# SHI-Labs/Prompt-Free-Diffusion

Measured on NVIDIA H100. Metric: 512x512 images/sec @ 50 DDIM steps, higher is better.
Workload: dtype fp16

## Files before the change

include/pfd_b200.h:

```cpp
#ifndef PFD_B200_H_
#define PFD_B200_H_

#include <stdint.h>

#ifdef __cplusplus
extern "C" {
#endif

#define PFD_ABI_VERSION 2
#if defined(__GNUC__)
#define PFD_API __attribute__((visibility("default")))
#else
#define PFD_API
#endif
#define PFD_MAX_SEG 3

enum {
  PFD_ACT_NONE = 0,
  PFD_ACT_SILU = 1,
  PFD_ACT_GELU = 2,
  PFD_ACT_RELU = 3,
  PFD_ACT_GEGLU = 4
};

PFD_API int pfd_version(void);
PFD_API const char* pfd_last_error(void);
PFD_API int64_t pfd_launch_count(void);
PFD_API int pfd_set_option(const char* name, int32_t value);

typedef struct pfd_gemm_desc {
  int32_t nseg;
  int32_t taps[PFD_MAX_SEG];
  int32_t a_c[PFD_MAX_SEG];
  const void* a_ptr[PFD_MAX_SEG];
  int64_t a_sx[PFD_MAX_SEG];
  int64_t a_sy[PFD_MAX_SEG];
  int64_t a_sn[PFD_MAX_SEG];
  int32_t in_w, in_h;
  int32_t stride;
  int32_t W, H, NB;

  const void* b_ptr;
  int32_t N;
  int64_t K;
  int64_t b_batch_stride;

  float alpha;
  int32_t act;
  const void* bias;
  const void* rowadd;
  int64_t rowadd_ld;
  const void* residual;

  void* out;
  int64_t so_n1, so_n0, so_y, so_x, so_c1, so_c0;
  int32_t ndiv, cdiv;
  int32_t bn_force;
  int32_t tap_off;
  void* stream;
} pfd_gemm_desc;

PFD_API int pfd_gemm_f16(const pfd_gemm_desc* d);
PFD_API int pfd_groupnorm_f16(const void* x1, int32_t c1, const void* x2, int32_t c2, int32_t NB,
                      int64_t HW, int32_t groups, const void* gamma, const void* beta, float eps,
                      int32_t silu, void* out, float* ws, int32_t zero_ws, void* stream);

// ... 161 lines not shown
```

pfd_b200/autokl.py:

```python
from __future__ import annotations

from typing import Optional

import torch
import torch.nn as nn

from . import native as nv
from .modules import Container, Conv2d, GroupNorm, pk_conv3, pk_conv3_small, pk_lin, pk_mat, pk_norm


def Normalize(c):
    return GroupNorm(32, c, eps=1e-6, affine=True)


class ResnetBlock(nn.Module):

    def __init__(self, in_channels, out_channels=None):
        super().__init__()
        out_channels = out_channels or in_channels
        self.in_channels, self.out_channels = in_channels, out_channels
        self.norm1 = Normalize(in_channels)
        self.conv1 = Conv2d(in_channels, out_channels, 3, padding=1)
        self.norm2 = Normalize(out_channels)
        self.dropout = nn.Dropout(0.0)
        self.conv2 = Conv2d(out_channels, out_channels, 3, padding=1)
        if in_channels != out_channels:
            self.nin_shortcut = Conv2d(in_channels, out_channels, 1)


class AttnBlock(nn.Module):

# ... 148 lines not shown
        if out_posterior:
            return DiagonalGaussianDistribution(mom, zc)
        noise = torch.randn((B, zc, mom.shape[1], mom.shape[2])).to(mom.device)
        return nv.vae_posterior(mom, zc, noise=noise, scale=post_scale, want=("sample",))["sample"]

    @torch.no_grad()
    def decode(self, z: torch.Tensor, pre_scale: float = 1.0) -> torch.Tensor:
        dec = self.decoder
        B, Cz, H, W = z.shape
        nv.gn_reset()
        zc = nv.nchw_to_nhwc(z if z.dtype == torch.float32 else z.to(torch.float16), cpad=8)
        wq, bq = pk_lin(self.post_quant_conv)
        h = nv.linear(zc.reshape(B * H * W, 8), wq, bq, alpha=pre_scale).reshape(B, H, W, 8)
        w, b = cached_conv_in(dec.conv_in, Cz)
        h = nv.conv3x3_im2col(h, w, b)
        h = run_vae_resnet(dec.mid.block_1, h)
        h = run_vae_attn(dec.mid.attn_1, h)
        h = run_vae_resnet(dec.mid.block_2, h)
        for lvl in reversed(range(dec.num_resolutions)):
            up = dec.up[lvl]
            for rb in up.block:
                h = run_vae_resnet(rb, h)
            if lvl != 0:
                w, b = pk_conv3(up.upsample.conv)
                h = nv.conv3x3(nv.upsample2x(h), w, b)
        g, b = pk_norm(dec.norm_out)
        h = nv.groupnorm(h, g, b, dec.norm_out.eps, silu=True)
        w, b = pk_conv3(dec.conv_out)
        h = nv.conv3x3(h, w, b)
        return nv.nhwc_to_nchw(h, dec.out_ch, mul=0.5, add=0.5, lo=0.0, hi=1.0)

    def forward(self, z):
        return self.decode(z)


class DiagonalGaussianDistribution(object):

    def __init__(self, moments: torch.Tensor, zc: int):
        self._mom, self._zc = moments, zc
        o = nv.vae_posterior(moments, zc, want=("mean", "logvar", "std"))
        self.mean, self.logvar, self.std = o["mean"], o["logvar"], o["std"]
        self.deterministic = False

    def sample(self):
        noise = torch.randn(self.mean.shape).to(self.mean.device)
        return nv.vae_posterior(self._mom, self._zc, noise=noise, want=("sample",))["sample"]

    def mode(self):
# ... 13 lines not shown
```

pfd_b200/csrc/gemm_tc.cu:

```cuda
#include <cuda.h>
#include <cuda_fp16.h>
#include <cuda_runtime.h>
#include <math.h>
#include <string.h>

#include "../../include/pfd_b200.h"
#include "common.h"
#include "ptx.cuh"
#include "wgmma.cuh"

namespace pfd {

constexpr int BM = 128;
constexpr int BK = 64;
constexpr int WG_K = 16;
constexpr int GEMM_THREADS = 384;
constexpr int STAGE_A_BYTES = BM * BK * 2;
constexpr int SMEM_BUDGET = 232448;
constexpr int SMEM_FIXED = 1024 + 256;

struct alignas(64) GemmParams {
  CUtensorMap tmA[PFD_MAX_SEG];
  CUtensorMap tmB;
  int nseg;
  int taps[PFD_MAX_SEG];
  int chunks[PFD_MAX_SEG];
  int a_c[PFD_MAX_SEG];
  int stride;
  int tap_off;
  int bw, bh, bn;
  int tiles_w, tiles_h, tiles_nb, n_tiles;
  int W, H, NB, N;
  int b_batched;
  int num_kb;
  int splits;
  int kb_per_split;
  float* ws;
  float alpha;
  int act;
  const __half* bias;
  const __half* rowadd;
  const __half* residual;
  __half* out;
  long long so_n1, so_n0, so_y, so_x, so_c1, so_c0;
  long long rowadd_ld;
  int ndiv, cdiv;
  int vec_ok;
};

constexpr int STORE_THREADS = 96;

template <int BN>
// ... 63 lines not shown

__device__ __forceinline__ __half2 geglu_pair(const float* v, const float* g, float alpha, uint32_t bv, uint32_t bg) {
  const __half2 a = __floats2half2_rn(fmaf(v[0], alpha, h2lo(bv)), fmaf(v[1], alpha, h2hi(bv)));
  const float2 gf = __half22float2(__floats2half2_rn(fmaf(g[0], alpha, h2lo(bg)), fmaf(g[1], alpha, h2hi(bg))));
  return __hmul2(a, __floats2half2_rn(gelu_sig(gf.x), gelu_sig(gf.y)));
}

struct WorkItem {
  int tile, kb0, kb1, slot;
};
__device__ __forceinline__ bool gemm_work(const GemmParams& p, int wi, int total_tiles, WorkItem& w) {
  const int G = gridDim.x, c = blockIdx.x;
  const int work = c + wi * G;
  if (work >= total_tiles * p.splits) return false;
  w.tile = work % total_tiles;
  w.slot = work / total_tiles;
  w.kb0 = w.slot * p.kb_per_split;
  w.kb1 = min(p.num_kb, w.kb0 + p.kb_per_split);
  return true;
}

struct TileOrigin {
  int x0, y0, n0, lbw, lbh;
};
__device__ __forceinline__ TileOrigin tile_origin(const GemmParams& p, int m_tile) {
  TileOrigin o;
  o.x0 = (m_tile % p.tiles_w) * p.bw;
  o.y0 = ((m_tile / p.tiles_w) % p.tiles_h) * p.bh;
  o.n0 = (m_tile / (p.tiles_w * p.tiles_h)) * p.bn;
  o.lbw = __ffs(p.bw) - 1;
  o.lbh = __ffs(p.bh) - 1;
  return o;
}
struct TileRow {
  int x, y, n;
  bool valid;
};
__device__ __forceinline__ TileRow tile_row(const GemmParams& p, const TileOrigin& o, int row) {
  TileRow r;
  r.x = o.x0 + (row & (p.bw - 1));
  r.y = o.y0 + ((row >> o.lbw) & (p.bh - 1));
  r.n = o.n0 + (row >> (o.lbw + o.lbh));
  r.valid = (r.x < p.W) && (r.y < p.H) && (r.n < p.NB);
  return r;
}
__device__ __forceinline__ long long out_row_off(const GemmParams& p, const TileRow& r) {
  return (long long)(r.n / p.ndiv) * p.so_n1 + (long long)(r.n % p.ndiv) * p.so_n0 + (long long)r.y * p.so_y +
         (long long)r.x * p.so_x;
}
__device__ __forceinline__ long long out_col_off(const GemmParams& p, int c) {
  return p.cdiv >= p.N ? (long long)c * p.so_c0 : (long long)(c / p.cdiv) * p.so_c1 + (long long)(c % p.cdiv) * p.so_c0;
}

template <int BN>
__device__ __forceinline__ void gemm_load_bias(const GemmParams& p, int tile, uint32_t (&bias)[BN / 8]) {
  const int col0 = (tile % p.n_tiles) * BN + 2 * (threadIdx.x & 3);
#pragma unroll
  for (int j = 0; j < BN / 8; ++j) bias[j] = (p.bias && col0 + 8 * j < p.N) ? ldg_h2(p.bias + col0 + 8 * j) : 0u;
}

template <int BN, bool GEGLU>
__device__ __forceinline__ void gemm_stage_tile(const GemmParams& p, const float (&acc)[BN / 2],
                                                const uint32_t (&bias)[BN / 8], int cw, int tile, uint8_t* cbuf) {
  constexpr int C_PITCH = GemmCfg<BN>::C_PITCH;
  const int wl = (threadIdx.x >> 5) & 3, lane = threadIdx.x & 31;
  const int n_tile = tile % p.n_tiles;
  const TileOrigin org = tile_origin(p, tile / p.n_tiles);
  const int n_out = GEGLU ? p.N / 2 : p.N;
  const int col_base = n_tile * (GEGLU ? BN / 2 : BN);
  const int cq = 2 * (lane & 3);
  int rows[2];
// ... 92 lines not shown
#pragma unroll 1
    for (int pass0 = 0; pass0 < NPASS; pass0 += STORE_BATCH) {
#pragma unroll
      for (int b = 0; b < STORE_BATCH; ++b) {
        const int row = r0 + (pass0 + b) * RPP;
        const long long off = (col_ok && row < BM) ? row_off(row) : -1;
        if (off < 0) continue;
        uint4 v = *reinterpret_cast<const uint4*>(src + (pass0 + b) * (RPP * C_PITCH));
        if (add_res) {
          __half2* h = reinterpret_cast<__half2*>(&v);
          const __half2* r = reinterpret_cast<const __half2*>(&res[b]);
#pragma unroll
          for (int k = 0; k < 4; ++k) h[k] = __hadd2(h[k], r[k]);
        }
        *reinterpret_cast<uint4*>(p.out + off) = v;
      }
      if (add_res && pass0 + STORE_BATCH < NPASS) load_batch(pass0 + STORE_BATCH);
    }
  };

  if (line_tile) {
    const int rows_in = p.W - org.x0;
    TileRow first;
    first.x = org.x0; first.y = org.y0; first.n = org.n0;
    const long long base = out_row_off(p, first) + col_off;
    const long long so_x = p.so_x;
    store_rows([&](int row) { return row < rows_in ? base + row * so_x : -1ll; });
  } else {
    store_rows([&](int row) {
      const long long ro = rowoff[row];
      return ro >= 0 ? ro + col_off : -1ll;
    });
  }
}

template <int BN>
__device__ __forceinline__ void gemm_epilogue(const GemmParams& p, const float (&acc)[BN / 2], int cw, int tile,
                                              int split, int m_tiles) {
  const int wl = (threadIdx.x >> 5) & 3, lane = threadIdx.x & 31;
  const int n_tile = tile % p.n_tiles;
  const int m_tile = tile / p.n_tiles;
  const TileOrigin org = tile_origin(p, m_tile);
  const bool geglu = (p.act == PFD_ACT_GEGLU);
  const int n_out = geglu ? p.N / 2 : p.N;
  const int col_base = n_tile * (geglu ? BN / 2 : BN);
  const int cq = 2 * (lane & 3);
  int rows[2];
// ... 89 lines not shown
  const uint32_t bars = base + STAGES * Cfg::STAGE_BYTES + Cfg::C_BYTES;
  auto full_bar = [&](int s) { return bars + 8u * s; };
  auto empty_bar = [&](int s) { return bars + 8u * (STAGES + s); };
  const uint32_t c_full = bars + 16u * STAGES, c_empty = c_full + 8u;

  const int wg = threadIdx.x >> 7;
  const bool staged = p.vec_ok && p.splits == 1;

  if (threadIdx.x == 0) {
    for (int s = 0; s < p.nseg; ++s) tma_prefetch_desc(&p.tmA[s]);
    tma_prefetch_desc(&p.tmB);
    for (int s = 0; s < STAGES; ++s) {
      mbar_init(full_bar(s), 1);
      mbar_init(empty_bar(s), 8);
    }
    mbar_init(c_full, 8);
    mbar_init(c_empty, STORE_THREADS / 32);
    mbar_fence_init();
  }
  __syncthreads();
  pdl_wait();
  pdl_launch_dependents();

  const int m_tiles = p.tiles_w * p.tiles_h * p.tiles_nb;
  const int total_tiles = m_tiles * p.n_tiles;

  if (wg == 0) {
    setmaxnreg_dec<Cfg::PRODUCER_REGS>();
    if (threadIdx.x >= 32 && staged) {
      uint32_t c_phase = 0;
      WorkItem w;
      for (int wi = 0; gemm_work(p, wi, total_tiles, w); ++wi) {
        if (p.act == PFD_ACT_GEGLU) gemm_store_tile<BN, true>(p, w.tile, cbuf, rowoff + (c_phase ? BM : 0), c_full, c_phase);
        else gemm_store_tile<BN, false>(p, w.tile, cbuf, rowoff + (c_phase ? BM : 0), c_full, c_phase);
        __syncwarp();
        if ((threadIdx.x & 31) == 0) mbar_arrive(c_empty);
        c_phase ^= 1u;
      }
    } else if (threadIdx.x == 0) {
      int stage = 0;
      uint32_t phase = 0;
      WorkItem w;
      for (int wi = 0; gemm_work(p, wi, total_tiles, w); ++wi) {
        const int tile = w.tile, kb_begin = w.kb0, kb_end = w.kb1;
        const int n_tile = tile % p.n_tiles;
        const int m_tile = tile / p.n_tiles;
        const int tx = m_tile % p.tiles_w;
        const int ty = (m_tile / p.tiles_w) % p.tiles_h;
        const int tn = m_tile / (p.tiles_w * p.tiles_h);
        const int x0 = tx * p.bw * p.stride;
        const int y0 = ty * p.bh * p.stride;
        const int n0 = tn * p.bn;
        const int bcoord = p.b_batched ? n0 : 0;
        int kofs = 0;
        int kbi = 0;
        for (int s = 0; s < p.nseg; ++s) {
          const int ntap = p.taps[s];
          for (int t = 0; t < ntap; ++t) {
            const int dy = (ntap == 9) ? (t / 3 - 1 + p.tap_off) : 0;
            const int dx = (ntap == 9) ? (t % 3 - 1 + p.tap_off) : 0;
            for (int j = 0; j < p.chunks[s]; ++j, ++kbi) {
              if (kbi < kb_begin || kbi >= kb_end) continue;
              mbar_wait(empty_bar(stage), phase ^ 1u);
              mbar_expect_tx(full_bar(stage), Cfg::STAGE_BYTES);
              tma_load_4d(smemA + stage * STAGE_A_BYTES, &p.tmA[s], full_bar(stage), j * BK, x0 + dx, y0 + dy, n0);
              tma_load_3d(smemB + stage * Cfg::STAGE_B_BYTES, &p.tmB, full_bar(stage), kofs + j * BK, n_tile * BN,
                          bcoord);
              if (++stage == STAGES) {
                stage = 0;
                phase ^= 1u;
              }
            }
            kofs += p.a_c[s];
          }
        }
      }
    }
  } else {
    setmaxnreg_inc<Cfg::CONSUMER_REGS>();
    const int cw = wg - 1;
    const bool arrive_lane = (threadIdx.x & 31) == 0;
    int stage = 0;
    uint32_t phase = 0, c_phase = 0;
// ... 22 lines not shown
        }
      }
      wgmma_wait<0>();
      if (prev >= 0 && arrive_lane) mbar_arrive(empty_bar(prev));
      if (staged) {
        if (!Cfg::BIAS_EARLY) gemm_load_bias<BN>(p, w.tile, bias);
        mbar_wait(c_empty, c_phase ^ 1u);
        if (p.act == PFD_ACT_GEGLU) gemm_stage_tile<BN, true>(p, acc, bias, cw, w.tile, cbuf);
        else gemm_stage_tile<BN, false>(p, acc, bias, cw, w.tile, cbuf);
        __syncwarp();
        if (arrive_lane) mbar_arrive(c_full);
        c_phase ^= 1u;
      } else {
        gemm_epilogue<BN>(p, acc, cw, w.tile, w.slot, m_tiles);
      }
    }
  }
}

__global__ void __launch_bounds__(256)
splitk_finish_kernel(const __grid_constant__ GemmParams p) {
  pdl_wait();
  pdl_launch_dependents();
  const int m_tiles = p.tiles_w * p.tiles_h * p.tiles_nb;
  const long long rows_pad = (long long)m_tiles * BM;
  const int vecs = p.N / 8;
  const long long total = rows_pad * vecs;
  for (long long i = (long long)blockIdx.x * blockDim.x + threadIdx.x; i < total; i += (long long)gridDim.x * blockDim.x) {
    const int v = (int)(i % vecs);
    const long long prow = i / vecs;
    const TileRow r = tile_row(p, tile_origin(p, (int)(prow / BM)), (int)(prow % BM));
    if (!r.valid) continue;
    const int col = v * 8;
    float acc[8];
#pragma unroll
    for (int k = 0; k < 8; ++k) acc[k] = 0.f;
    for (int s = 0; s < p.splits; ++s) {
      const float4* src = reinterpret_cast<const float4*>(p.ws + ((long long)s * rows_pad + prow) * p.N + col);
      const float4 a = __ldg(src), b = __ldg(src + 1);
      acc[0] += a.x; acc[1] += a.y; acc[2] += a.z; acc[3] += a.w;
      acc[4] += b.x; acc[5] += b.y; acc[6] += b.z; acc[7] += b.w;
    }
    uint4 bv = make_uint4(0, 0, 0, 0), rv = bv;
    if (p.bias) bv = __ldg(reinterpret_cast<const uint4*>(p.bias + col));
    if (p.rowadd) rv = __ldg(reinterpret_cast<const uint4*>(p.rowadd + (long long)r.n * p.rowadd_ld + col));
    const uint32_t* b2 = &bv.x;
    const uint32_t* r2 = &rv.x;
// ... 20 lines not shown
        const long long off = row_off + out_col_off(p, col + k);
        __half h = __float2half_rn(acc[k]);
        if (p.residual) h = __hadd(h, p.residual[off]);
        p.out[off] = h;
      }
    }
  }
}

constexpr size_t SPLITK_WS_BYTES = (64ull << 20) - 4096;

static inline long long cdivll(long long a, long long b) { return (a + b - 1) / b; }

template <int BN>
static int launch_gemm(const GemmParams& p, int grid, cudaStream_t stream) {
  using Cfg = GemmCfg<BN>;
  static int trace = -1;
  if (trace < 0) {
    const char* e = getenv("PFD_GEMM_TRACE");
    trace = (e && e[0] == '1') ? 1 : 0;
  }
  if (trace)
    fprintf(stderr, "GEMMTRACE M=%lld N=%d K=%d nseg=%d taps=%d stride=%d act=%d bias=%d res=%d rowadd=%d BN=%d "
            "splits=%d grid=%d batched=%d vec=%d plain=%d\n", (long long)p.W * p.H * p.NB, p.N, p.num_kb * BK,
            p.nseg, p.taps[0], p.stride, p.act, p.bias != nullptr, p.residual != nullptr, p.rowadd != nullptr, BN,
            p.splits, grid, p.b_batched, p.vec_ok, (int)(p.cdiv >= p.N));
  if (int rc = smem_opt_in<gemm_wgmma_kernel<BN>>(Cfg::SMEM_BYTES, "gemm_wgmma_kernel")) return rc;
  launch_k(gemm_wgmma_kernel<BN>, dim3(grid), dim3(GEMM_THREADS), Cfg::SMEM_BYTES, stream, p);
  return check_launch("pfd_gemm_f16");
}

}

using namespace pfd;

extern "C" PFD_API int pfd_gemm_f16(const pfd_gemm_desc* d) {
  if (!d) return set_error("pfd_gemm_f16: null descriptor");
  if (d->nseg < 1 || d->nseg > PFD_MAX_SEG) return set_error("pfd_gemm_f16: nseg %d out of range", d->nseg);
  if (d->N <= 0 || d->N % 8) return set_error("pfd_gemm_f16: N=%d must be a positive multiple of 8", d->N);
  if (d->K % 8) return set_error("pfd_gemm_f16: K pitch %lld must be a multiple of 8", (long long)d->K);
  if (d->W <= 0 || d->H <= 0 || d->NB <= 0) return set_error("pfd_gemm_f16: empty output raster");
  if (d->stride != 1 && d->stride != 2) return set_error("pfd_gemm_f16: stride %d unsupported", d->stride);
  if (d->tap_off != 0 && d->tap_off != 1) return set_error("pfd_gemm_f16: tap_off %d unsupported", d->tap_off);
  if (!d->out || !d->b_ptr) return set_error("pfd_gemm_f16: null out/b pointer");
  long long ktot = 0;
  for (int s = 0; s < d->nseg; ++s) {
    if (d->taps[s] != 1 && d->taps[s] != 9) return set_error("pfd_gemm_f16: taps[%d]=%d", s, d->taps[s]);
    if (d->a_c[s] <= 0 || d->a_c[s] % 8) return set_error("pfd_gemm_f16: a_c[%d]=%d must be a multiple of 8", s, d->a_c[s]);
    if (!d->a_ptr[s]) return set_error("pfd_gemm_f16: a_ptr[%d] is null", s);
    if ((reinterpret_cast<uintptr_t>(d->a_ptr[s]) & 15) || (d->a_sx[s] % 8) || (d->a_sy[s] % 8) || (d->a_sn[s] % 8))
      return set_error("pfd_gemm_f16: A segment %d not 16-byte aligned/strided", s);
    ktot += (long long)d->taps[s] * d->a_c[s];
  }
  if (ktot > d->K) return set_error("pfd_gemm_f16: segments cover K=%lld > pitch %lld", ktot, (long long)d->K);
  if (reinterpret_cast<uintptr_t>(d->b_ptr) & 15) return set_error("pfd_gemm_f16: B not 16-byte aligned");
  const bool geglu = d->act == PFD_ACT_GEGLU;

  GemmParams p;
  memset(&p, 0, sizeof(p));
  p.nseg = d->nseg;
  p.stride = d->stride;
  p.tap_off = d->tap_off;
  p.W = d->W; p.H = d->H; p.NB = d->NB; p.N = d->N;
  p.b_batched = d->b_batch_stride != 0;
  p.alpha = d->alpha;
  p.act = d->act;
  p.bias = static_cast<const __half*>(d->bias);
  p.rowadd = static_cast<const __half*>(d->rowadd);
  p.residual = static_cast<const __half*>(d->residual);
  p.rowadd_ld = d->rowadd_ld > 0 ? d->rowadd_ld : d->N;
  p.out = static_cast<__half*>(d->out);
  p.so_n1 = d->so_n1; p.so_n0 = d->so_n0; p.so_y = d->so_y; p.so_x = d->so_x;
  p.so_c1 = d->so_c1; p.so_c0 = d->so_c0;
  p.ndiv = d->ndiv > 0 ? d->ndiv : 1;
  p.cdiv = d->cdiv > 0 ? d->cdiv : (1 << 30);
  p.vec_ok = (d->so_c0 == 1) && (p.cdiv % 8 == 0) && (d->so_n1 % 8 == 0) && (d->so_n0 % 8 == 0) &&
             (d->so_y % 8 == 0) && (d->so_x % 8 == 0) && (d->so_c1 % 8 == 0) &&
             ((reinterpret_cast<uintptr_t>(d->out) & 15) == 0) &&
             ((reinterpret_cast<uintptr_t>(d->residual) & 15) == 0);
  if ((reinterpret_cast<uintptr_t>(d->bias) & 15) || (reinterpret_cast<uintptr_t>(d->rowadd) & 15) || (d->rowadd_ld % 8))
    return set_error("pfd_gemm_f16: bias/rowadd must be 16-byte aligned");

  int bw = 128, bh = 1, bn = 1;
  if (!p.b_batched) {
    long long best = -1;
    for (int cw = 128; cw >= 1; cw >>= 1) {
      if (cw * d->stride > 256) continue;
      for (int ch = 128 / cw; ch >= 1; ch >>= 1) {
        if (ch * d->stride > 256) continue;
        int cn = 128 / (cw * ch);
        long long cost = cdivll(d->W, cw) * cdivll(d->H, ch) * cdivll(d->NB, cn);
        if (best < 0 || cost < best) {
          best = cost; bw = cw; bh = ch; bn = cn;
        }
      }
    }
  }
  p.bw = bw; p.bh = bh; p.bn = bn;
  p.tiles_w = (int)cdivll(d->W, bw);
  p.tiles_h = (int)cdivll(d->H, bh);
  p.tiles_nb = (int)cdivll(d->NB, bn);
  const long long m_tiles = (long long)p.tiles_w * p.tiles_h * p.tiles_nb;

  bool short_k_plain = !p.b_batched && !geglu;
  int kb_count = 0;
  for (int s = 0; s < d->nseg; ++s) {
    if (d->taps[s] != 1) short_k_plain = false;
    kb_count += d->taps[s] * ((d->a_c[s] + BK - 1) / BK);
  }
  short_k_plain = short_k_plain && kb_count <= 40;
  const int cands[5] = {256, 192, 160, 128, 64};
  int BNsel = 128;
  double best_cost = -1;
  const int sms = plan_sms();
  for (int i = 0; i < 5; ++i) {
    const int bn_c = cands[i];
    if (geglu && (d->N % bn_c)) continue;
    if (d->bn_force && d->bn_force != bn_c) continue;
    if (short_k_plain && !d->bn_force && bn_c != 64) continue;
    const long long nt = cdivll(d->N, bn_c);
    const long long tiles = m_tiles * nt;
    const double waves = (double)cdivll(tiles, sms);
    const double cost = waves * (bn_c + 24);
    if (best_cost < 0 || cost < best_cost - 1e-9) {
      best_cost = cost; BNsel = bn_c;
    }
  }
  if (best_cost < 0) return set_error("pfd_gemm_f16: no valid N tile (bn_force=%d, N=%d, geglu=%d)", d->bn_force, d->N, (int)geglu);
  p.n_tiles = (int)cdivll(d->N, BNsel);
  p.splits = 1;

  int num_kb = 0;
  for (int s = 0; s < d->nseg; ++s) {
    p.taps[s] = d->taps[s];
    p.a_c[s] = d->a_c[s];
    p.chunks[s] = (d->a_c[s] + BK - 1) / BK;
    num_kb += p.taps[s] * p.chunks[s];
    cuuint64_t dims[4] = {(cuuint64_t)d->a_c[s], (cuuint64_t)d->in_w, (cuuint64_t)d->in_h, (cuuint64_t)d->NB};
    cuuint64_t strides[3] = {(cuuint64_t)d->a_sx[s] * 2, (cuuint64_t)d->a_sy[s] * 2, (cuuint64_t)d->a_sn[s] * 2};
    cuuint32_t box[4] = {(cuuint32_t)BK, (cuuint32_t)(bw * d->stride), (cuuint32_t)(bh * d->stride), (cuuint32_t)bn};
    cuuint32_t estr[4] = {1, (cuuint32_t)d->stride, (cuuint32_t)d->stride, 1};
    if (int rc = encode_tensor_map_f16(&p.tmA[s], d->a_ptr[s], 4, dims, strides, box, estr, "A")) return rc;
// ... 11 lines not shown
        break;
      }
    const long long nt_sk = cdivll(d->N, bn_sk);
    const long long tiles_sk = m_tiles * nt_sk;
    if (tiles_sk * 2 <= sms) {
      int splits = (int)(sms / tiles_sk);
      if (splits > 8) splits = 8;
      if (splits > num_kb / 8) splits = num_kb / 8;
      const size_t need = (size_t)splits * (size_t)m_tiles * BM * (size_t)d->N * sizeof(float);
      if (splits >= 2 && need <= SPLITK_WS_BYTES) {
        float* ws = skws;
        if (ws) {
          BNsel = bn_sk;
          p.n_tiles = (int)nt_sk;
          p.splits = splits;
          p.kb_per_split = (num_kb + splits - 1) / splits;
          p.splits = (num_kb + p.kb_per_split - 1) / p.kb_per_split;
          p.ws = ws;
        }
      }
    }
  }
  {
    const long long nbatch = p.b_batched ? d->NB : 1;
    cuuint64_t dims[3] = {(cuuint64_t)d->K, (cuuint64_t)d->N, (cuuint64_t)nbatch};
    const long long bs = p.b_batched ? d->b_batch_stride : (long long)d->K * d->N;
    cuuint64_t strides[2] = {(cuuint64_t)d->K * 2, (cuuint64_t)bs * 2};
    cuuint32_t box[3] = {(cuuint32_t)BK, (cuuint32_t)BNsel, 1};
    cuuint32_t estr[3] = {1, 1, 1};
    if (int rc = encode_tensor_map_f16(&p.tmB, d->b_ptr, 3, dims, strides, box, estr, "B")) return rc;
  }
  const long long total = m_tiles * p.n_tiles * p.splits;
  int grid = (int)(total < sms ? total : sms);
  int rc;
  switch (BNsel) {
    case 64: rc = launch_gemm<64>(p, grid, st); break;
    case 128: rc = launch_gemm<128>(p, grid, st); break;
    case 160: rc = launch_gemm<160>(p, grid, st); break;
    case 192: rc = launch_gemm<192>(p, grid, st); break;
    default: rc = launch_gemm<256>(p, grid, st); break;
  }
  if (rc || p.splits == 1) return rc;
  const long long vec_items = m_tiles * BM * (long long)(d->N / 8);
  long long fgrid = (vec_items + 255) / 256;
  if (fgrid > 8LL * sms) fgrid = 8LL * sms;
  launch_k(splitk_finish_kernel, dim3((unsigned)fgrid), dim3(256), 0, st, p);
  return check_launch("pfd_gemm_f16(split-K finish)");
// ... 2 lines not shown
```

pfd_b200/modules.py:

```python
from __future__ import annotations

from typing import Callable, Optional, Sequence, Tuple

import torch
import torch.nn as nn

from .graphs import generation, watch


class _Holder:
    def forward(self, *a, **k):
        raise RuntimeError(f"{type(self).__name__} is a parameter holder: pfd_b200 computes through "
                           "the CUDA C-ABI kernels only (no torch fallback)")


class Conv2d(_Holder, nn.Conv2d):
    pass


class Linear(_Holder, nn.Linear):
    pass


class GroupNorm(_Holder, nn.GroupNorm):
# ... 68 lines not shown
    o, i, kh, kw = w.shape
    if cin is not None and cin > i:
        w = torch.cat([w, w.new_zeros((o, cin - i, kh, kw))], 1)
    return w.permute(0, 2, 3, 1).reshape(o, -1).contiguous()


def pk_conv3(conv: nn.Conv2d, skip: Optional[nn.Conv2d] = None) -> Tuple[torch.Tensor, Optional[torch.Tensor]]:
    def build():
        w = pack_conv(conv.weight)
        b = fp16(conv.bias)
        if skip is not None:
            ws = fp16(skip.weight).reshape(skip.weight.shape[0], -1)
            w = torch.cat([w, ws], 1).contiguous()
            if skip.bias is not None:
                b = (conv.bias.detach().float() + skip.bias.detach().float()).to(torch.float16).contiguous()
        if w.shape[0] % 8:
            w = pad_rows(w)
            b = pad_rows(b) if b is not None else None
        return w, b
    params = [conv.weight, conv.bias] + ([skip.weight, skip.bias] if skip is not None else [])
    return cached(conv, "conv3" + ("+skip" if skip is not None else ""), params, build)


def pk_conv3_small(conv: nn.Conv2d) -> Tuple[torch.Tensor, Optional[torch.Tensor]]:
    def build():
        w = pad_cols(pack_conv(conv.weight))
        b = fp16(conv.bias)
        if w.shape[0] % 8:
            w, b = pad_rows(w), (pad_rows(b) if b is not None else None)
        return w, b
    return cached(conv, "conv3s", [conv.weight, conv.bias], build)


def pk_mat(mod: nn.Module, weight: torch.Tensor, bias: Optional[torch.Tensor], key: str = "mat",
           rows: Optional[slice] = None) -> Tuple[torch.Tensor, Optional[torch.Tensor]]:
    def build():
        w = fp16(weight).reshape(weight.shape[0], -1)
        b = fp16(bias)
        if rows is not None:
            w = w[rows].contiguous()
            b = b[rows].contiguous() if b is not None else None
        if w.shape[1] % 8:
            w = pad_cols(w)
        if w.shape[0] % 8:
            w, b = pad_rows(w), (pad_rows(b) if b is not None else None)
        return w, b
# ... 14 lines not shown
```

pfd_b200/native.py:

```python
from __future__ import annotations

import ctypes
import os
import re
from ctypes import POINTER, c_char_p, c_float, c_int32, c_int64, c_uint32, c_void_p
from typing import Dict, List, Optional, Sequence, Tuple

import torch

_HERE = os.path.dirname(os.path.abspath(__file__))
LIB_PATH = os.environ.get("PFD_B200_LIB") or os.path.join(_HERE, "libpfd_b200.so")
HEADER = os.path.join(_HERE, os.pardir, "include", "pfd_b200.h")

PFD_MAX_SEG = 3
ACT_NONE, ACT_SILU, ACT_GELU, ACT_RELU, ACT_GEGLU = 0, 1, 2, 3, 4
PFD_KSAMPLER_NCOEF = 6
PFD_HED_MAX_SIDES = 5
PFD_PIDINET_SIDE_PARAMS = 161
PFD_MLSD_TOPK = 200
PFD_OPENPOSE_MAX_PEAKS = 128
PFD_OPENPOSE_MAX_PERSONS = 17 * PFD_OPENPOSE_MAX_PEAKS


class GemmDesc(ctypes.Structure):
    _fields_ = [
        ("nseg", c_int32),
        ("taps", c_int32 * PFD_MAX_SEG),
        ("a_c", c_int32 * PFD_MAX_SEG),
        ("a_ptr", c_void_p * PFD_MAX_SEG),
        ("a_sx", c_int64 * PFD_MAX_SEG),
        ("a_sy", c_int64 * PFD_MAX_SEG),
        ("a_sn", c_int64 * PFD_MAX_SEG),
        ("in_w", c_int32), ("in_h", c_int32),
        ("stride", c_int32),
        ("W", c_int32), ("H", c_int32), ("NB", c_int32),
        ("b_ptr", c_void_p),
        ("N", c_int32),
        ("K", c_int64),
        ("b_batch_stride", c_int64),
        ("alpha", c_float),
        ("act", c_int32),
        ("bias", c_void_p),
        ("rowadd", c_void_p),
        ("rowadd_ld", c_int64),
        ("residual", c_void_p),
        ("out", c_void_p),
        ("so_n1", c_int64), ("so_n0", c_int64), ("so_y", c_int64), ("so_x", c_int64),
        ("so_c1", c_int64), ("so_c0", c_int64),
        ("ndiv", c_int32), ("cdiv", c_int32),
        ("bn_force", c_int32),
        ("tap_off", c_int32),
        ("stream", c_void_p),
    ]


class DevicePtr(c_void_p):

    @classmethod
    def from_param(cls, obj):
        if isinstance(obj, torch.Tensor):
# ... 110 lines not shown
def _chk16(t: torch.Tensor, name: str) -> None:
    if t.dtype != torch.float16 or not t.is_cuda:
        raise RuntimeError(f"{name}: expected a CUDA fp16 tensor, got {t.dtype} on {t.device}")


def _chk32(t: torch.Tensor, name: str) -> None:
    if t.dtype != torch.float32 or not t.is_cuda or not t.is_contiguous():
        raise RuntimeError(f"{name}: expected a contiguous CUDA fp32 tensor, got {t.dtype} on {t.device}")


def _chk_image(x: torch.Tensor, what: str) -> Tuple[torch.Tensor, int]:
    if x.dim() != 4 or x.shape[1] != 3 or not x.is_cuda or x.dtype not in (torch.float16, torch.float32):
        raise RuntimeError(f"{what}: expected a CUDA fp16/fp32 [B,3,H,W] image, got {tuple(x.shape)} {x.dtype} "
                           f"{x.device}")
    return x.contiguous(), int(x.dtype == torch.float32)


def gemm_raw(segs: Sequence[Tuple[torch.Tensor, int, int, Tuple[int, int, int]]], *, in_w: int,
             in_h: int, stride: int, W: int, H: int, NB: int, w: torch.Tensor, N: int, K: int,
             b_batch_stride: int = 0, alpha: float = 1.0, act: int = ACT_NONE,
             bias: Optional[torch.Tensor] = None, rowadd: Optional[torch.Tensor] = None,
             residual: Optional[torch.Tensor] = None, out: torch.Tensor,
             so: Tuple[int, int, int, int, int, int], ndiv: int = 1, cdiv: int = 0,
             bn_force: int = 0, tap_off: int = 0) -> None:
    d = GemmDesc()
    d.nseg = len(segs)
    for i, (t, taps, c, (sx, sy, sn)) in enumerate(segs):
        _chk16(t, f"A[{i}]")
        d.taps[i] = taps
        d.a_c[i] = c
        d.a_ptr[i] = t.data_ptr()
        d.a_sx[i], d.a_sy[i], d.a_sn[i] = sx, sy, sn
    d.in_w, d.in_h, d.stride = in_w, in_h, stride
    d.W, d.H, d.NB = W, H, NB
    _chk16(w, "B")
    d.b_ptr = w.data_ptr()
    d.N, d.K, d.b_batch_stride = N, K, b_batch_stride
    d.alpha, d.act = alpha, act
    d.bias = _p(bias)
    d.rowadd = _p(rowadd)
    d.rowadd_ld = rowadd.stride(0) if rowadd is not None else 0
    d.residual = _p(residual)
    d.out = out.data_ptr()
    d.so_n1, d.so_n0, d.so_y, d.so_x, d.so_c1, d.so_c0 = so
    d.ndiv, d.cdiv = ndiv, cdiv
    d.bn_force = bn_force
    d.tap_off = tap_off
    d.stream = stream_ptr()
    _check(load().pfd_gemm_f16(ctypes.byref(d)), "pfd_gemm_f16")


def linear(x: torch.Tensor, w: torch.Tensor, bias: Optional[torch.Tensor] = None, *, act: int = ACT_NONE,
           residual: Optional[torch.Tensor] = None, out: Optional[torch.Tensor] = None,
           alpha: float = 1.0, x2: Optional[torch.Tensor] = None, bn_force: int = 0) -> torch.Tensor:
    M, K1 = x.shape
    N = w.shape[0]
    n_out = N // 2 if act == ACT_GEGLU else N
    if out is None:
        out = torch.empty((M, n_out), device=x.device, dtype=torch.float16)
    segs = [(x, 1, K1, (x.stride(0), x.stride(0) * M, x.stride(0) * M))]
# ... 21 lines not shown
    tile = torch.arange(n2 // bn, device=w.device).reshape(-1, 1)
    j = torch.arange(h, device=w.device).reshape(1, -1)
    src = torch.stack([tile * h + j, inner + tile * h + j], dim=1).reshape(-1)
    wp = w.index_select(0, src).contiguous()
    bp = b.index_select(0, src).contiguous() if b is not None else None
    return wp, bp, bn


def conv3x3(x: torch.Tensor, w: torch.Tensor, bias: Optional[torch.Tensor] = None, *, stride: int = 1,
            rowadd: Optional[torch.Tensor] = None, act: int = ACT_NONE,
            residual: Optional[torch.Tensor] = None, out: Optional[torch.Tensor] = None,
            skip: Sequence[torch.Tensor] = (), tap_off: int = 0) -> torch.Tensor:
    NB, H, W, C = x.shape
    Ho, Wo = (H - 1 - tap_off) // stride + 1, (W - 1 - tap_off) // stride + 1
    N = w.shape[0]
    if out is None:
        out = torch.empty((NB, Ho, Wo, N), device=x.device, dtype=torch.float16)
    segs = [(x, 9, C, (x.stride(2), x.stride(1), x.stride(0)))]
    for s in skip:
        segs.append((s, 1, s.shape[3], (s.stride(2), s.stride(1), s.stride(0))))
    gemm_raw(segs, in_w=W, in_h=H, stride=stride, W=Wo, H=Ho, NB=NB, w=w, N=N, K=w.stride(0), act=act,
             bias=bias, rowadd=rowadd, residual=residual, out=out,
             so=(out.stride(0), 0, out.stride(1), out.stride(2), 0, 1), tap_off=tap_off)
    return out


def conv1x1(x: torch.Tensor, w: torch.Tensor, bias: Optional[torch.Tensor] = None, *, act: int = ACT_NONE,
            residual: Optional[torch.Tensor] = None, out: Optional[torch.Tensor] = None,
            x2: Optional[torch.Tensor] = None) -> torch.Tensor:
    NB, H, W, C = x.shape
    N = w.shape[0]
    if out is None:
        out = torch.empty((NB, H, W, N), device=x.device, dtype=torch.float16)
    r = residual.reshape(NB * H * W, -1) if residual is not None else None
    linear(x.reshape(NB * H * W, C), w, bias, act=act, residual=r, out=out.reshape(NB * H * W, N),
           x2=None if x2 is None else x2.reshape(NB * H * W, -1))
    return out


def conv1x1_into(x: torch.Tensor, w: torch.Tensor, bias: Optional[torch.Tensor], out: torch.Tensor, *,
                 act: int = ACT_NONE) -> torch.Tensor:
    NB, H, W, C = x.shape
    gemm_raw([(x, 1, C, (x.stride(2), x.stride(1), x.stride(0)))], in_w=W, in_h=H, stride=1, W=W, H=H, NB=NB, w=w,
             N=w.shape[0], K=w.stride(0), act=act, bias=bias, out=out,
             so=(out.stride(0), 0, out.stride(1), out.stride(2), 0, 1))
    return out
# ... 677 lines not shown
```

pfd_b200/unet.py:

```python
from __future__ import annotations

from typing import Dict, List, Optional, Sequence, Tuple

import torch
import torch.nn as nn

from . import native as nv
from . import attention as att
from .attention import attend, ceil8, project_heads, project_heads_fused, project_vt_swapped
from .modules import (Conv2d, GroupNorm, IndexedSequential, LayerNorm, Linear, cached, pk_conv3,
                      pk_conv3_small, pk_lin, pk_mat, pk_norm)


class ResBlock(nn.Module):

    def __init__(self, channels, emb_channels, dropout=0.0, out_channels=None, **_):
        super().__init__()
        self.channels = channels
        self.out_channels = out_channels or channels
        self.in_layers = IndexedSequential(GroupNorm(32, channels), nn.SiLU(),
                                           Conv2d(channels, self.out_channels, 3, padding=1))
        self.emb_layers = IndexedSequential(nn.SiLU(), Linear(emb_channels, self.out_channels))
        self.out_layers = IndexedSequential(GroupNorm(32, self.out_channels), nn.SiLU(), nn.Dropout(p=dropout),
                                            Conv2d(self.out_channels, self.out_channels, 3, padding=1))
        if self.out_channels == channels:
            self.skip_connection = nn.Identity()
        else:
            self.skip_connection = Conv2d(channels, self.out_channels, 1)


class Downsample(nn.Module):

    def __init__(self, channels, out_channels=None):
        super().__init__()
# ... 249 lines not shown
        self.parameter_group = {'global': self.time_embed, 'data': self.data_blocks,
                                'context': self.context_blocks}

    def get_d_head_n_heads(self, ch):
        if self.num_head_channels is None:
            return ch // self.num_heads, self.num_heads
        return self.num_head_channels, ch // self.num_head_channels

    def resblocks(self) -> List[ResBlock]:
        return [blk[0] for blk in self.data_blocks if isinstance(blk[0], ResBlock)]

    def prepare_context(self, context: torch.Tensor) -> List[Tuple[torch.Tensor, torch.Tensor]]:
        return [context_kv(cb[0], context) for cb in self.context_blocks]

    def run_data_block(self, idx: int, h, h2, embs: Dict[int, torch.Tensor]):
        layer = self.data_blocks[idx][0]
        if isinstance(layer, ResBlock):
            return run_resblock(layer, h, h2, embs[idx])
        assert h2 is None
        if isinstance(layer, Downsample):
            w, b = pk_conv3(layer.op)
            return nv.conv3x3(h, w, b, stride=2)
        if isinstance(layer, Upsample):
            w, b = pk_conv3(layer.conv)
            return nv.conv3x3(nv.upsample2x(h), w, b)
        if isinstance(layer, IndexedSequential):
            g, b = pk_norm(layer[0])
            hn = nv.groupnorm(h, g, b, layer[0].eps, silu=True)
            w, bb = pk_conv3(layer[2])
            return nv.conv3x3(hn, w, bb)
        if isinstance(layer, Conv2d):
            w, b = pk_conv3_small(layer)
            return nv.conv3x3_im2col(h, w, b)
        raise RuntimeError(f"unknown data block {type(layer)}")

    def apply(self, x: torch.Tensor, timesteps: torch.Tensor, context: torch.Tensor,
              control: Optional[List[torch.Tensor]] = None,
              kv: Optional[List[Tuple[torch.Tensor, torch.Tensor]]] = None,
              mixed_contexts: Optional[List[Tuple[torch.Tensor, float]]] = None) -> torch.Tensor:
        x = x.to(torch.float16)
        context = context.to(torch.float16).contiguous()
        B = x.shape[0]
        nv.gn_reset()
        silu_emb = time_embed_silu(self.time_embed, timesteps, self.model_channels)
        rbs = [i for i, blk in enumerate(self.data_blocks) if isinstance(blk[0], ResBlock)]
        emb_list = batched_emb_layers(self, [self.data_blocks[i][0] for i in rbs], silu_emb)
        embs = dict(zip(rbs, emb_list))
        if kv is None and mixed_contexts is None:
# ... 36 lines not shown
```

Before: 3.772.

## Fuse nearest upsample into 3x3 conv via four-phase 2x2 folded weights

Replaces the nearest-neighbour upsample followed by a 3x3 conv with a single implicit GEMM. For each of the four output phases, the 3x3 kernel is folded into a 2x2 kernel applied to the low-resolution input, and the phase selects both the weight batch and the output offset. This avoids materialising the 4x-larger upsampled tensor and cuts the conv K dimension from 9 to 4 taps per channel. It also changes the BN heuristic for short-K plain GEMMs (128 when N>=640 with enough tiles) and excludes BN=256 for up2x, and it adds phase indexing overhead to the tile scheduling.

Result: faster. 3.843, median of 6 (+1.9%).

```diff
diff --git a/include/pfd_b200.h b/include/pfd_b200.h
--- a/include/pfd_b200.h
+++ b/include/pfd_b200.h
@@ -42,6 +42,7 @@
 
   const void* b_ptr;
   int32_t N;
+  int32_t up2x;
   int64_t K;
   int64_t b_batch_stride;
 
diff --git a/pfd_b200/autokl.py b/pfd_b200/autokl.py
--- a/pfd_b200/autokl.py
+++ b/pfd_b200/autokl.py
@@ -6,7 +6,7 @@
 import torch.nn as nn
 
 from . import native as nv
-from .modules import Container, Conv2d, GroupNorm, pk_conv3, pk_conv3_small, pk_lin, pk_mat, pk_norm
+from .modules import Container, Conv2d, GroupNorm, pk_conv3, pk_conv3_small, pk_conv3_up2x, pk_lin, pk_mat, pk_norm
 
 
 def Normalize(c):
@@ -201,8 +201,8 @@
             for rb in up.block:
                 h = run_vae_resnet(rb, h)
             if lvl != 0:
-                w, b = pk_conv3(up.upsample.conv)
-                h = nv.conv3x3(nv.upsample2x(h), w, b)
+                w, b = pk_conv3_up2x(up.upsample.conv)
+                h = nv.conv3x3_up2x(h, w, b)
         g, b = pk_norm(dec.norm_out)
         h = nv.groupnorm(h, g, b, dec.norm_out.eps, silu=True)
         w, b = pk_conv3(dec.conv_out)
diff --git a/pfd_b200/csrc/gemm_tc.cu b/pfd_b200/csrc/gemm_tc.cu
--- a/pfd_b200/csrc/gemm_tc.cu
+++ b/pfd_b200/csrc/gemm_tc.cu
@@ -28,6 +28,8 @@
   int a_c[PFD_MAX_SEG];
   int stride;
   int tap_off;
+  int phases;
+  long long ph_sy, ph_sx;
   int bw, bh, bn;
   int tiles_w, tiles_h, tiles_nb, n_tiles;
   int W, H, NB, N;
@@ -137,9 +139,17 @@
 
 struct TileOrigin {
   int x0, y0, n0, lbw, lbh;
+  long long obase;
 };
 __device__ __forceinline__ TileOrigin tile_origin(const GemmParams& p, int m_tile) {
   TileOrigin o;
+  o.obase = 0;
+  if (p.phases > 1) {
+    const int per_phase = p.tiles_w * p.tiles_h * p.tiles_nb;
+    const int ph = m_tile / per_phase;
+    m_tile -= ph * per_phase;
+    o.obase = ((ph & 2) ? p.ph_sy : 0ll) + ((ph & 1) ? p.ph_sx : 0ll);
+  }
   o.x0 = (m_tile % p.tiles_w) * p.bw;
   o.y0 = ((m_tile / p.tiles_w) % p.tiles_h) * p.bh;
   o.n0 = (m_tile / (p.tiles_w * p.tiles_h)) * p.bn;
@@ -150,6 +160,7 @@
 struct TileRow {
   int x, y, n;
   bool valid;
+  long long obase;
 };
 __device__ __forceinline__ TileRow tile_row(const GemmParams& p, const TileOrigin& o, int row) {
   TileRow r;
@@ -157,11 +168,12 @@
   r.y = o.y0 + ((row >> o.lbw) & (p.bh - 1));
   r.n = o.n0 + (row >> (o.lbw + o.lbh));
   r.valid = (r.x < p.W) && (r.y < p.H) && (r.n < p.NB);
+  r.obase = o.obase;
   return r;
 }
 __device__ __forceinline__ long long out_row_off(const GemmParams& p, const TileRow& r) {
-  return (long long)(r.n / p.ndiv) * p.so_n1 + (long long)(r.n % p.ndiv) * p.so_n0 + (long long)r.y * p.so_y +
-         (long long)r.x * p.so_x;
+  return r.obase + (long long)(r.n / p.ndiv) * p.so_n1 + (long long)(r.n % p.ndiv) * p.so_n0 +
+         (long long)r.y * p.so_y + (long long)r.x * p.so_x;
 }
 __device__ __forceinline__ long long out_col_off(const GemmParams& p, int c) {
   return p.cdiv >= p.N ? (long long)c * p.so_c0 : (long long)(c / p.cdiv) * p.so_c1 + (long long)(c % p.cdiv) * p.so_c0;
@@ -300,7 +312,7 @@
   if (line_tile) {
     const int rows_in = p.W - org.x0;
     TileRow first;
-    first.x = org.x0; first.y = org.y0; first.n = org.n0;
+    first.x = org.x0; first.y = org.y0; first.n = org.n0; first.obase = org.obase;
     const long long base = out_row_off(p, first) + col_off;
     const long long so_x = p.so_x;
     store_rows([&](int row) { return row < rows_in ? base + row * so_x : -1ll; });
@@ -436,7 +448,7 @@
   pdl_wait();
   pdl_launch_dependents();
 
-  const int m_tiles = p.tiles_w * p.tiles_h * p.tiles_nb;
+  const int m_tiles = p.tiles_w * p.tiles_h * p.tiles_nb * p.phases;
   const int total_tiles = m_tiles * p.n_tiles;
 
   if (wg == 0) {
@@ -458,21 +470,23 @@
       for (int wi = 0; gemm_work(p, wi, total_tiles, w); ++wi) {
         const int tile = w.tile, kb_begin = w.kb0, kb_end = w.kb1;
         const int n_tile = tile % p.n_tiles;
-        const int m_tile = tile / p.n_tiles;
+        const int per_phase = p.tiles_w * p.tiles_h * p.tiles_nb;
+        const int ph = (tile / p.n_tiles) / per_phase;
+        const int m_tile = (tile / p.n_tiles) % per_phase;
         const int tx = m_tile % p.tiles_w;
         const int ty = (m_tile / p.tiles_w) % p.tiles_h;
         const int tn = m_tile / (p.tiles_w * p.tiles_h);
         const int x0 = tx * p.bw * p.stride;
         const int y0 = ty * p.bh * p.stride;
         const int n0 = tn * p.bn;
-        const int bcoord = p.b_batched ? n0 : 0;
+        const int bcoord = p.b_batched ? n0 : ph;
         int kofs = 0;
         int kbi = 0;
         for (int s = 0; s < p.nseg; ++s) {
           const int ntap = p.taps[s];
           for (int t = 0; t < ntap; ++t) {
-            const int dy = (ntap == 9) ? (t / 3 - 1 + p.tap_off) : 0;
-            const int dx = (ntap == 9) ? (t % 3 - 1 + p.tap_off) : 0;
+            const int dy = (ntap == 9) ? (t / 3 - 1 + p.tap_off) : (ntap == 4) ? (t / 2 - 1 + (ph >> 1)) : 0;
+            const int dx = (ntap == 9) ? (t % 3 - 1 + p.tap_off) : (ntap == 4) ? (t % 2 - 1 + (ph & 1)) : 0;
             for (int j = 0; j < p.chunks[s]; ++j, ++kbi) {
               if (kbi < kb_begin || kbi >= kb_end) continue;
               mbar_wait(empty_bar(stage), phase ^ 1u);
@@ -541,7 +555,7 @@
 splitk_finish_kernel(const __grid_constant__ GemmParams p) {
   pdl_wait();
   pdl_launch_dependents();
-  const int m_tiles = p.tiles_w * p.tiles_h * p.tiles_nb;
+  const int m_tiles = p.tiles_w * p.tiles_h * p.tiles_nb * p.phases;
   const long long rows_pad = (long long)m_tiles * BM;
   const int vecs = p.N / 8;
   const long long total = rows_pad * vecs;
@@ -608,9 +622,9 @@
   }
   if (trace)
     fprintf(stderr, "GEMMTRACE M=%lld N=%d K=%d nseg=%d taps=%d stride=%d act=%d bias=%d res=%d rowadd=%d BN=%d "
-            "splits=%d grid=%d batched=%d vec=%d plain=%d\n", (long long)p.W * p.H * p.NB, p.N, p.num_kb * BK,
-            p.nseg, p.taps[0], p.stride, p.act, p.bias != nullptr, p.residual != nullptr, p.rowadd != nullptr, BN,
-            p.splits, grid, p.b_batched, p.vec_ok, (int)(p.cdiv >= p.N));
+            "splits=%d grid=%d batched=%d vec=%d plain=%d phases=%d\n", (long long)p.W * p.H * p.NB * p.phases, p.N,
+            p.num_kb * BK, p.nseg, p.taps[0], p.stride, p.act, p.bias != nullptr, p.residual != nullptr, p.rowadd != nullptr, BN,
+            p.splits, grid, p.b_batched, p.vec_ok, (int)(p.cdiv >= p.N), p.phases);
   if (int rc = smem_opt_in<gemm_wgmma_kernel<BN>>(Cfg::SMEM_BYTES, "gemm_wgmma_kernel")) return rc;
   launch_k(gemm_wgmma_kernel<BN>, dim3(grid), dim3(GEMM_THREADS), Cfg::SMEM_BYTES, stream, p);
   return check_launch("pfd_gemm_f16");
@@ -628,10 +642,17 @@
   if (d->W <= 0 || d->H <= 0 || d->NB <= 0) return set_error("pfd_gemm_f16: empty output raster");
   if (d->stride != 1 && d->stride != 2) return set_error("pfd_gemm_f16: stride %d unsupported", d->stride);
   if (d->tap_off != 0 && d->tap_off != 1) return set_error("pfd_gemm_f16: tap_off %d unsupported", d->tap_off);
+  if (d->up2x != 0 && d->up2x != 1) return set_error("pfd_gemm_f16: up2x %d unsupported", d->up2x);
+  if (d->up2x && (d->stride != 1 || d->tap_off != 0 || d->b_batch_stride != 0 || d->W != 2 * d->in_w ||
+                  d->H != 2 * d->in_h))
+    return set_error("pfd_gemm_f16: up2x needs stride 1, tap_off 0, shared weights and W, H = 2 in_w, 2 in_h "
+                     "(got stride %d, tap_off %d, W %d, H %d, in_w %d, in_h %d)", d->stride, d->tap_off, d->W, d->H,
+                     d->in_w, d->in_h);
   if (!d->out || !d->b_ptr) return set_error("pfd_gemm_f16: null out/b pointer");
   long long ktot = 0;
   for (int s = 0; s < d->nseg; ++s) {
-    if (d->taps[s] != 1 && d->taps[s] != 9) return set_error("pfd_gemm_f16: taps[%d]=%d", s, d->taps[s]);
+    if (d->up2x ? d->taps[s] != 4 : (d->taps[s] != 1 && d->taps[s] != 9))
+      return set_error("pfd_gemm_f16: taps[%d]=%d (up2x %d)", s, d->taps[s], d->up2x);
     if (d->a_c[s] <= 0 || d->a_c[s] % 8) return set_error("pfd_gemm_f16: a_c[%d]=%d must be a multiple of 8", s, d->a_c[s]);
     if (!d->a_ptr[s]) return set_error("pfd_gemm_f16: a_ptr[%d] is null", s);
     if ((reinterpret_cast<uintptr_t>(d->a_ptr[s]) & 15) || (d->a_sx[s] % 8) || (d->a_sy[s] % 8) || (d->a_sn[s] % 8))
@@ -647,7 +668,9 @@
   p.nseg = d->nseg;
   p.stride = d->stride;
   p.tap_off = d->tap_off;
-  p.W = d->W; p.H = d->H; p.NB = d->NB; p.N = d->N;
+  p.phases = d->up2x ? 4 : 1;
+  const int sc = d->up2x ? 2 : 1;
+  p.W = d->W / sc; p.H = d->H / sc; p.NB = d->NB; p.N = d->N;
   p.b_batched = d->b_batch_stride != 0;
   p.alpha = d->alpha;
   p.act = d->act;
@@ -656,7 +679,9 @@
   p.residual = static_cast<const __half*>(d->residual);
   p.rowadd_ld = d->rowadd_ld > 0 ? d->rowadd_ld : d->N;
   p.out = static_cast<__half*>(d->out);
-  p.so_n1 = d->so_n1; p.so_n0 = d->so_n0; p.so_y = d->so_y; p.so_x = d->so_x;
+  p.so_n1 = d->so_n1; p.so_n0 = d->so_n0; p.so_y = d->so_y * sc; p.so_x = d->so_x * sc;
+  p.ph_sy = d->up2x ? d->so_y : 0;
+  p.ph_sx = d->up2x ? d->so_x : 0;
   p.so_c1 = d->so_c1; p.so_c0 = d->so_c0;
   p.ndiv = d->ndiv > 0 ? d->ndiv : 1;
   p.cdiv = d->cdiv > 0 ? d->cdiv : (1 << 30);
@@ -675,7 +700,7 @@
       for (int ch = 128 / cw; ch >= 1; ch >>= 1) {
         if (ch * d->stride > 256) continue;
         int cn = 128 / (cw * ch);
-        long long cost = cdivll(d->W, cw) * cdivll(d->H, ch) * cdivll(d->NB, cn);
+        long long cost = cdivll(p.W, cw) * cdivll(p.H, ch) * cdivll(d->NB, cn);
         if (best < 0 || cost < best) {
           best = cost; bw = cw; bh = ch; bn = cn;
         }
@@ -683,10 +708,10 @@
     }
   }
   p.bw = bw; p.bh = bh; p.bn = bn;
-  p.tiles_w = (int)cdivll(d->W, bw);
-  p.tiles_h = (int)cdivll(d->H, bh);
+  p.tiles_w = (int)cdivll(p.W, bw);
+  p.tiles_h = (int)cdivll(p.H, bh);
   p.tiles_nb = (int)cdivll(d->NB, bn);
-  const long long m_tiles = (long long)p.tiles_w * p.tiles_h * p.tiles_nb;
+  const long long m_tiles = (long long)p.tiles_w * p.tiles_h * p.tiles_nb * p.phases;
 
   bool short_k_plain = !p.b_batched && !geglu;
   int kb_count = 0;
@@ -695,6 +720,7 @@
     kb_count += d->taps[s] * ((d->a_c[s] + BK - 1) / BK);
   }
   short_k_plain = short_k_plain && kb_count <= 40;
+  const int short_k_bn = (!d->residual && d->N >= 640 && m_tiles >= 64) ? 128 : 64;
   const int cands[5] = {256, 192, 160, 128, 64};
   int BNsel = 128;
   double best_cost = -1;
@@ -703,7 +729,8 @@
     const int bn_c = cands[i];
     if (geglu && (d->N % bn_c)) continue;
     if (d->bn_force && d->bn_force != bn_c) continue;
-    if (short_k_plain && !d->bn_force && bn_c != 64) continue;
+    if (short_k_plain && !d->bn_force && bn_c != short_k_bn) continue;
+    if (d->up2x && !d->bn_force && bn_c == 256) continue;
     const long long nt = cdivll(d->N, bn_c);
     const long long tiles = m_tiles * nt;
     const double waves = (double)cdivll(tiles, sms);
@@ -761,7 +788,7 @@
     }
   }
   {
-    const long long nbatch = p.b_batched ? d->NB : 1;
+    const long long nbatch = p.b_batched ? d->NB : p.phases;
     cuuint64_t dims[3] = {(cuuint64_t)d->K, (cuuint64_t)d->N, (cuuint64_t)nbatch};
     const long long bs = p.b_batched ? d->b_batch_stride : (long long)d->K * d->N;
     cuuint64_t strides[2] = {(cuuint64_t)d->K * 2, (cuuint64_t)bs * 2};
diff --git a/pfd_b200/modules.py b/pfd_b200/modules.py
--- a/pfd_b200/modules.py
+++ b/pfd_b200/modules.py
@@ -114,6 +114,30 @@
     return cached(conv, "conv3" + ("+skip" if skip is not None else ""), params, build)
 
 
+UP2X_FOLD = (((0,), (1, 2)), ((0, 1), (2,)))
+
+
+def up2x_phase_weights(w: torch.Tensor) -> torch.Tensor:
+    f = torch.zeros((2, 2, 3), dtype=w.dtype, device=w.device)
+    for p in range(2):
+        for t in range(2):
+            f[p, t, list(UP2X_FOLD[p][t])] = 1
+    return torch.einsum("pyk,qxl,oikl->pqoiyx", f, f, w)
+
+
+def pk_conv3_up2x(conv: nn.Conv2d) -> Tuple[torch.Tensor, Optional[torch.Tensor]]:
+    def build():
+        w = up2x_phase_weights(fp16(conv.weight).float())
+        o, i = w.shape[2], w.shape[3]
+        w = w.permute(0, 1, 2, 4, 5, 3).reshape(4, o, 4 * i)
+        b = fp16(conv.bias)
+        if o % 8:
+            w = torch.cat([w, w.new_zeros((4, 8 - o % 8, 4 * i))], 1)
+            b = pad_rows(b) if b is not None else None
+        return w.to(torch.float16).contiguous(), b
+    return cached(conv, "conv3up2x", [conv.weight, conv.bias], build)
+
+
 def pk_conv3_small(conv: nn.Conv2d) -> Tuple[torch.Tensor, Optional[torch.Tensor]]:
     def build():
         w = pad_cols(pack_conv(conv.weight))
diff --git a/pfd_b200/native.py b/pfd_b200/native.py
--- a/pfd_b200/native.py
+++ b/pfd_b200/native.py
@@ -36,6 +36,7 @@
         ("W", c_int32), ("H", c_int32), ("NB", c_int32),
         ("b_ptr", c_void_p),
         ("N", c_int32),
+        ("up2x", c_int32),
         ("K", c_int64),
         ("b_batch_stride", c_int64),
         ("alpha", c_float),
@@ -192,7 +193,7 @@
              bias: Optional[torch.Tensor] = None, rowadd: Optional[torch.Tensor] = None,
              residual: Optional[torch.Tensor] = None, out: torch.Tensor,
              so: Tuple[int, int, int, int, int, int], ndiv: int = 1, cdiv: int = 0,
-             bn_force: int = 0, tap_off: int = 0) -> None:
+             bn_force: int = 0, tap_off: int = 0, up2x: int = 0) -> None:
     d = GemmDesc()
     d.nseg = len(segs)
     for i, (t, taps, c, (sx, sy, sn)) in enumerate(segs):
@@ -206,6 +207,7 @@
     _chk16(w, "B")
     d.b_ptr = w.data_ptr()
     d.N, d.K, d.b_batch_stride = N, K, b_batch_stride
+    d.up2x = up2x
     d.alpha, d.act = alpha, act
     d.bias = _p(bias)
     d.rowadd = _p(rowadd)
@@ -273,6 +275,18 @@
     gemm_raw(segs, in_w=W, in_h=H, stride=stride, W=Wo, H=Ho, NB=NB, w=w, N=N, K=w.stride(0), act=act,
              bias=bias, rowadd=rowadd, residual=residual, out=out,
              so=(out.stride(0), 0, out.stride(1), out.stride(2), 0, 1), tap_off=tap_off)
+    return out
+
+
+def conv3x3_up2x(x: torch.Tensor, w: torch.Tensor, bias: Optional[torch.Tensor] = None, *,
+                 out: Optional[torch.Tensor] = None) -> torch.Tensor:
+    NB, H, W, C = x.shape
+    N = w.shape[1]
+    if out is None:
+        out = torch.empty((NB, 2 * H, 2 * W, N), device=x.device, dtype=torch.float16)
+    gemm_raw([(x, 4, C, (x.stride(2), x.stride(1), x.stride(0)))], in_w=W, in_h=H, stride=1, W=2 * W, H=2 * H, NB=NB,
+             w=w, N=N, K=w.stride(1), bias=bias, out=out, so=(out.stride(0), 0, out.stride(1), out.stride(2), 0, 1),
+             up2x=1)
     return out
 
 
diff --git a/pfd_b200/unet.py b/pfd_b200/unet.py
--- a/pfd_b200/unet.py
+++ b/pfd_b200/unet.py
@@ -9,7 +9,7 @@
 from . import attention as att
 from .attention import attend, ceil8, project_heads, project_heads_fused, project_vt_swapped
 from .modules import (Conv2d, GroupNorm, IndexedSequential, LayerNorm, Linear, cached, pk_conv3,
-                      pk_conv3_small, pk_lin, pk_mat, pk_norm)
+                      pk_conv3_small, pk_conv3_up2x, pk_lin, pk_mat, pk_norm)
 
 
 class ResBlock(nn.Module):
@@ -305,8 +305,8 @@
             w, b = pk_conv3(layer.op)
             return nv.conv3x3(h, w, b, stride=2)
         if isinstance(layer, Upsample):
-            w, b = pk_conv3(layer.conv)
-            return nv.conv3x3(nv.upsample2x(h), w, b)
+            w, b = pk_conv3_up2x(layer.conv)
+            return nv.conv3x3_up2x(h, w, b)
         if isinstance(layer, IndexedSequential):
             g, b = pk_norm(layer[0])
             hn = nv.groupnorm(h, g, b, layer[0].eps, silu=True)
```
